# FrancisGregoryNg/Gaussian_Process_Optimization

Measured on AMD Instinct MI355X. Metric: GP fit+predict iters/sec at N=16384 D=8, higher is better.
Workload: dtype f64; 1 GPU; C3 (BASELINE.json configs[2]): N=16384, D=8 RBF iso, fit (K, Cholesky, alpha, LML) + predict mean/var at M=10000 candidates + EI arg-best; candidates_total=10000, candidates_this_rank=10000, entry_point=gp_fit_predict, kernel=RBF, fit=replicated on every rank (does not shard, SURVEY.md 8e), torch_imported=False, launcher=single process, emulate_fp64=0

## Files before the change

### gaussian_process_optimization_amd/_lib.py

```python
import ctypes
import os

import numpy as np

_HERE = os.path.dirname(os.path.abspath(__file__))
LIB_PATH = os.path.join(_HERE, "libgphip.so")

c_double_p = ctypes.POINTER(ctypes.c_double)
c_int64_p = ctypes.POINTER(ctypes.c_int64)
c_int_p = ctypes.POINTER(ctypes.c_int)

GP_KERNEL_RBF, GP_KERNEL_MATERN52 = 0, 1
GP_KERNEL_MATERN32, GP_KERNEL_EXPONENTIAL = 2, 3
GP_ACQ_EI, GP_ACQ_LCB, GP_ACQ_MPI = 0, 1, 2
GP_ERR_ARG, GP_ERR_HIP, GP_ERR_STATE, GP_ERR_RCCL, GP_ERR_NOT_PD_DIAG = -1, -2, -3, -4, -5

_vp = ctypes.c_void_p
SIGNATURES = [
    ("gp_last_error", ctypes.c_char_p, []),
    ("gp_version", ctypes.c_char_p, []),
    ("gp_device_count", ctypes.c_int, [c_int_p]),
    ("gp_device_info", ctypes.c_int, [ctypes.c_int, ctypes.c_char_p, ctypes.c_int, c_int_p, c_int64_p]),
    ("gp_create", ctypes.c_int, [ctypes.POINTER(_vp), ctypes.c_int]),
    ("gp_destroy", ctypes.c_int, [_vp]),
# ... 95 lines not shown
    ("gp_comm_info", ctypes.c_int, [_vp, c_int_p, c_int_p]),
    ("gp_comm_allgather_best", ctypes.c_int, [_vp, ctypes.c_double, ctypes.c_int64, c_double_p, c_int64_p]),
    ("gp_comm_bcast_fit", ctypes.c_int, [_vp, ctypes.c_int]),
    ("gp_comm_version", ctypes.c_int, [c_int_p]),
    ("gp_comm_selftest_fit_record", ctypes.c_int, [c_double_p, c_double_p, c_int_p]),
    ("gp_group_create", ctypes.c_int, [ctypes.POINTER(_vp), ctypes.c_int, c_int_p]),
    ("gp_group_destroy", ctypes.c_int, [_vp]),
    ("gp_group_info", ctypes.c_int, [_vp, c_int_p, c_int_p, ctypes.c_char_p, ctypes.c_int]),
    ("gp_group_member", ctypes.c_int, [_vp, ctypes.c_int, ctypes.POINTER(_vp)]),
    ("gp_group_set_data", ctypes.c_int, [_vp, c_double_p, c_double_p, ctypes.c_int64, ctypes.c_int, ctypes.c_int]),
    ("gp_group_set_params", ctypes.c_int, [_vp, ctypes.c_int, ctypes.c_int, ctypes.c_double, c_double_p, ctypes.c_double]),
    ("gp_group_set_gower", ctypes.c_int, [_vp, ctypes.c_int, c_int_p, c_double_p]),
    ("gp_group_set_option", ctypes.c_int, [_vp, ctypes.c_char_p, ctypes.c_int64]),
    ("gp_group_fit", ctypes.c_int, [_vp, ctypes.c_int, c_double_p, c_double_p, c_double_p]),
    ("gp_group_fmin", ctypes.c_int, [_vp, c_double_p]),
    ("gp_group_set_candidates", ctypes.c_int, [_vp, c_double_p, ctypes.c_int64]),
    ("gp_group_acq_argbest", ctypes.c_int, [_vp, ctypes.c_int, ctypes.c_double, ctypes.c_double, ctypes.c_double,
                                            ctypes.c_double, ctypes.c_int, c_int64_p, c_double_p]),
    ("gp_group_acq_lp_argbest", ctypes.c_int, [_vp, ctypes.c_int, ctypes.c_double, ctypes.c_double, ctypes.c_double,
                                               ctypes.c_double, ctypes.c_int, c_double_p, ctypes.c_int, c_double_p, c_double_p,
                                               ctypes.c_int, c_int64_p, ctypes.c_int, c_int64_p, c_double_p]),
    ("gp_group_acq_topk", ctypes.c_int, [_vp, ctypes.c_int, ctypes.c_double, ctypes.c_double, ctypes.c_double,
                                         ctypes.c_double, ctypes.c_int, ctypes.c_int, c_int64_p, c_double_p]),
    ("gp_merge_best", ctypes.c_int, [ctypes.c_int, c_double_p, c_int64_p, ctypes.c_int, c_int64_p, c_double_p]),
    ("gp_merge_topk", ctypes.c_int, [ctypes.c_int, c_double_p, c_int64_p, ctypes.c_int, ctypes.c_int, c_int64_p, c_double_p]),
    ("gp_last_phases", ctypes.c_int, [_vp, ctypes.c_int, ctypes.POINTER(ctypes.c_char_p), c_double_p, c_double_p,
                                      c_double_p]),
    ("gp_profile", ctypes.c_int, [_vp, ctypes.c_int]),
    ("gp_gemm_stats", ctypes.c_int, [_vp, c_int64_p, c_double_p, c_double_p]),
    ("gp_rns_stats", ctypes.c_int, [_vp, c_int64_p, c_double_p, c_double_p]),
    ("gp_gemm_busy", ctypes.c_int, [_vp, c_double_p]),
    ("gp_gemm_trace", ctypes.c_int, [_vp, ctypes.c_int, c_int64_p, c_int_p, c_double_p]),
    ("gp_synchronize", ctypes.c_int, [_vp]),
    ("gp_set_option", ctypes.c_int, [_vp, ctypes.c_char_p, ctypes.c_int64]),
]

_lib = None


def load_library():
    global _lib
    if _lib is not None:
        return _lib
    if not os.path.exists(LIB_PATH):
        raise RuntimeError(
            "libgphip.so is missing at %s: build it with `python -c 'import __graft_entry__ as g; g.build()'` "
            "(hipcc --offload-arch=gfx950). There is no CPU fallback." % LIB_PATH)
    lib = ctypes.CDLL(LIB_PATH)
    for name, restype, argtypes in SIGNATURES:
        fn = getattr(lib, name)
        fn.restype = restype
        fn.argtypes = argtypes
    _lib = lib
    return lib


def load():
    lib = load_library()
    n = ctypes.c_int(0)
    rc = lib.gp_device_count(ctypes.byref(n))
    if rc != 0 or n.value < 1:
        raise RuntimeError("gphip: no HIP device visible (%s). The GP path runs on MI355X only; "
                           "there is no CPU fallback." % lib.gp_last_error().decode())
    return lib


# ... 636 lines not shown

    def profile(self, on=True):
        check(self.lib, self.lib.gp_profile(self.h, int(on)), "gp_profile")

    def gemm_stats(self):
        n, ms, fl = ctypes.c_int64(), ctypes.c_double(), ctypes.c_double()
        check(self.lib, self.lib.gp_gemm_stats(self.h, ctypes.byref(n), ctypes.byref(ms), ctypes.byref(fl)),
              "gp_gemm_stats")
        return dict(launches=n.value, ms=ms.value, flops=fl.value)

    def rns_stats(self):
        n, ms, ops = ctypes.c_int64(), ctypes.c_double(), ctypes.c_double()
        check(self.lib, self.lib.gp_rns_stats(self.h, ctypes.byref(n), ctypes.byref(ms), ctypes.byref(ops)), "gp_rns_stats")
        return dict(launches=n.value, ms=ms.value, ops=ops.value)

    def gemm_busy(self):
        b = ctypes.c_double()
        check(self.lib, self.lib.gp_gemm_busy(self.h, ctypes.byref(b)), "gp_gemm_busy")
        return b.value

    def gemm_trace(self, cap=100000):
        tiles = np.empty(cap, dtype=np.int64)
        K = np.empty(cap, dtype=np.int32)
        ms = np.empty(cap)
        n = self.lib.gp_gemm_trace(self.h, cap, tiles.ctypes.data_as(c_int64_p), K.ctypes.data_as(c_int_p), dptr(ms))
        return tiles[:n], K[:n], ms[:n]

    def synchronize(self):
        check(self.lib, self.lib.gp_synchronize(self.h), "gp_synchronize")

    def set_option(self, name, value):
        check(self.lib, self.lib.gp_set_option(self.h, name.encode(), int(value)), "gp_set_option")

    def comm_unique_id(self):
        buf = ctypes.create_string_buffer(128)
        check(self.lib, self.lib.gp_comm_unique_id(buf), "gp_comm_unique_id")
        return buf.raw

    def comm_version(self):
        v = ctypes.c_int()
        check(self.lib, self.lib.gp_comm_version(ctypes.byref(v)), "gp_comm_version")
        return v.value

    def comm_init(self, uid, rank, nranks):
        check(self.lib, self.lib.gp_comm_init(self.h, uid, int(rank), int(nranks)), "gp_comm_init")

    def comm_info(self):
        r, n = ctypes.c_int(), ctypes.c_int()
        check(self.lib, self.lib.gp_comm_info(self.h, ctypes.byref(r), ctypes.byref(n)), "gp_comm_info")
        return r.value, n.value

    def comm_allgather_best(self, val, idx, nranks):
        vals = np.empty(nranks)
        idxs = np.empty(nranks, dtype=np.int64)
        check(self.lib, self.lib.gp_comm_allgather_best(self.h, float(val), int(idx), dptr(vals),
                                                        idxs.ctypes.data_as(c_int64_p)), "gp_comm_allgather_best")
        return vals, idxs

    def comm_allgather_topk(self, vals, idxs, nranks):
        vals = as_f64(vals, 1)
        idxs = np.ascontiguousarray(idxs, dtype=np.int64)
        k = vals.size
        av = np.empty(nranks * k)
        ai = np.empty(nranks * k, dtype=np.int64)
        check(self.lib, self.lib.gp_comm_allgather_topk(self.h, k, dptr(vals), idxs.ctypes.data_as(c_int64_p), dptr(av),
                                                        ai.ctypes.data_as(c_int64_p)), "gp_comm_allgather_topk")
# ... 106 lines not shown
```

### gaussian_process_optimization_amd/csrc/api_core.hip

```cpp
#include "api_internal.h"

thread_local std::string g_err;

static thread_local bool g_note_set = false;
static thread_local std::string g_note_msg;

int fail(int code, const char *fmt, ...) {
    char buf[512];
    va_list ap;
    va_start(ap, fmt);
    vsnprintf(buf, sizeof buf, fmt, ap);
    va_end(ap);
    g_err = buf;
    if (g_note_set) {
        g_err += " [after: " + g_note_msg + "]";
        g_note_set = false;
    }
    return code;
}

void gp_note_hip(hipError_t e, const char *what, const char *file, int line) {
    if (e == hipSuccess || g_note_set) return;
    char buf[512];
    snprintf(buf, sizeof buf, "%s -> %s (%s:%d)", what, hipGetErrorString(e), file, line);
    g_note_msg = buf;
    g_note_set = true;
}
int gp_pending_error() {
    if (!g_note_set) return 0;
    g_note_set = false;
    return fail(GP_ERR_HIP, "%s", g_note_msg.c_str());
}
void gp_clear_stale_note() { g_note_set = false; }
// ... 64 lines not shown
            int rp = reserve;
            if (const char *e = getenv("GPHIP_PRED_RESERVE")) rp = atoi(e);
            rc = make_bulk_stream(device, rp, &d.pred);
            if (rc) return rc;
        }
    }
    *out = d;
    return 0;
}

int phase_begin(gp_ctx *g, const char *name, double flops, double bytes) {
    if (g->nphases >= MAX_PHASES) return -1;
    Phase &p = g->phases[g->nphases];
    p.name = name;
    p.flops = flops;
    p.bytes = bytes;
    if (!p.used) {
        hipEventCreate(&p.e0);
        hipEventCreate(&p.e1);
        p.used = true;
    }
    GP_NOTE(hipEventRecord(p.e0, g->s));
    return g->nphases++;
}
void phase_end(gp_ctx *g, int id) {
    if (id >= 0) GP_NOTE(hipEventRecord(g->phases[id].e1, g->s));
}

void gemm(gp_ctx *g, hipStream_t s, int mode, double *C, long ldc, const double *A, long lda, const double *B, long ldb, int b_mul, int K, TileSet ts, const GemmOpt &o) {
    if (o.batch <= 0 || o.members <= 0) return;
    const long n = tileset_count(ts) * (o.batch / o.members), n_all = tileset_count(ts) * o.batch;
    if (n <= 0 || K <= 0) return;
    GemmOpt oo = o;
    if (n >= 1024 && !oo.stagger) oo.stagger = g->stagger;
    if (n >= 1024 && g->waves8) oo.waves8 = 1;
    if (oo.inplace && g->trsm_rows64 && !oo.waves8) oo.rows64 = g->trsm_rows64;
    const int small_thr = (s == g->s_panel) ? g->chain_small_below : g->small_below;
    if (small_thr > 0 && n < small_thr && !oo.inplace) oo.small = 1;
    if (g->pair_tri && (oo.small || (oo.waves8 && g->pair_tri >= 2)) && o.k_end_tri && !ts.tri && !o.tile_list && ts.c1 - ts.c0 >= 2)
        oo.pair = 1;
    hipEvent_t e0 = nullptr, e1 = nullptr;
    const bool small_sym = mode == 1 && oo.small && !oo.pair && !oo.rows64;
    const bool timed = g->profiling && (g->profile_class == 1 ? small_sym :
                       (n >= g->profile_min_tiles &&
                        (g->profile_min_tiles < 1024 || (mode == 1 && oo.waves8 && !oo.small))));
    if (timed) {
        if (g->gemm_ev_used + 2 > g->gemm_events.size()) {
            hipEvent_t a, b;
            hipEventCreate(&a);
            hipEventCreate(&b);
            g->gemm_events.push_back(a);
            g->gemm_events.push_back(b);
        }
        e0 = g->gemm_events[g->gemm_ev_used++];
        e1 = g->gemm_events[g->gemm_ev_used++];
        GP_NOTE(hipEventRecord(e0, s));
        g->gemm_tiles.push_back(n_all);
        g->gemm_K.push_back((o.k_tri || o.k_end_tri) ? -K : K);
    }
    if (g->supertile > 1 && !o.tile_list && !o.k_end_tri && o.batch == 1 && tileset_count(ts) >= 2048) {
        const std::array<int, 5> key{ts.r0, ts.r1, ts.c0, ts.c1, ts.tri};
        auto it = g->tile_lists.find(key);
        if (it == g->tile_lists.end()) {
            std::vector<short> l = build_tile_list(ts, g->supertile);
            DevBuf<short> d;
            if (d.alloc((long)l.size()) == hipSuccess) {
                hipMemcpy(d, l.data(), l.size() * sizeof(short), hipMemcpyHostToDevice);
                it = g->tile_lists.emplace(key, std::move(d)).first;
// ... 159 lines not shown
    delete g;
    return 0;
}

enum OptShape { OPT_RANGE, OPT_FLOOR, OPT_BOOL, OPT_RAW };
struct OptDesc {
    const char *name;
    int gp_ctx::*field;
    OptShape shape;
    int lo, hi;
};
static const OptDesc g_options[] = {
    {"panel_tiles", &gp_ctx::panel_tiles, OPT_RANGE, 1, 64},
    {"inner_tiles", &gp_ctx::inner_tiles, OPT_RANGE, 1, 2},
    {"inner_min_rows", &gp_ctx::inner_min_rows, OPT_FLOOR, 0},
    {"own_keep_per_row", &gp_ctx::own_keep_per_row, OPT_FLOOR, 0},
    {"own_keep_pipe_pct", &gp_ctx::own_keep_pipe_pct, OPT_RANGE, 0, 400},
    {"own_keep_base", &gp_ctx::own_keep_base, OPT_FLOOR, 0},
    {"lookahead", &gp_ctx::lookahead, OPT_BOOL},
    {"lookahead_min_tiles", &gp_ctx::lookahead_min_tiles, OPT_FLOOR, 0},
    {"pipe_start_pct", &gp_ctx::pipe_start_pct, OPT_RANGE, -1, 100},
    {"small_below", &gp_ctx::small_below, OPT_RAW},
    {"pipe_stages_grad", &gp_ctx::pipe_stages_grad, OPT_FLOOR, 0},
    {"pipe_start_pct_grad", &gp_ctx::pipe_start_pct_grad, OPT_RANGE, 0, 100},
    {"pipe_stages", &gp_ctx::pipe_stages, OPT_FLOOR, 0},
    {"lauum_panels", &gp_ctx::lauum_panels, OPT_RAW},
    {"side_alpha", &gp_ctx::side_alpha, OPT_RAW},
    {"pair_panels", &gp_ctx::pair_panels, OPT_BOOL},
    {"pair_tri", &gp_ctx::pair_tri, OPT_RAW},
    {"fmin_direct", &gp_ctx::fmin_direct, OPT_RAW},
    {"chain_small_below", &gp_ctx::chain_small_below, OPT_RAW},
    {"waves8", &gp_ctx::waves8, OPT_BOOL},
    {"stagger", &gp_ctx::stagger, OPT_RAW},
    {"trsm_rows64", &gp_ctx::trsm_rows64, OPT_RAW},
    {"rns_group_fit", &gp_ctx::rns_group_fit, OPT_RANGE, 1, 16},
    {"rns_group", &gp_ctx::rns_group, OPT_RANGE, 1, 16},
    {"emulate_fit", &gp_ctx::emulate_fit, OPT_BOOL},
    {"emulate_fp64", &gp_ctx::emulate_fp64, OPT_BOOL},
    {"rows_build", &gp_ctx::rows_build, OPT_RANGE, -1, 1},
    {"rows_nt", &gp_ctx::rows_nt, OPT_RANGE, -1, 1},
    {"rows_wide", &gp_ctx::rows_wide, OPT_BOOL},
};

static int store_option(gp_ctx *g, const OptDesc &o, int64_t value) {
    if (o.shape == OPT_RANGE && (value < o.lo || value > o.hi))
        return fail(GP_ERR_ARG, "%s out of range [%d, %d]", o.name, o.lo, o.hi);
    if (o.shape == OPT_FLOOR && value < o.lo) return fail(GP_ERR_ARG, "%s < %d", o.name, o.lo);
    if (o.shape == OPT_FLOOR) value = std::min<int64_t>(value, 1 << 20);
    if (o.shape == OPT_BOOL) value = value ? 1 : 0;
    g->*o.field = (int)value;
    return 0;
}

extern "C" int gp_set_option(gp_t *g, const char *name, int64_t value) {
    if (!g || !name) return fail(GP_ERR_ARG, "null argument");
    GP_DEAD_CHECK(g);
    for (const OptDesc &o : g_options) {
        if (strcmp(name, o.name)) continue;
        int rc = store_option(g, o, value);
        if (rc) return rc;
        if (o.field == &gp_ctx::lauum_panels) {
            g->wi_valid = false;
            g->li_valid = false;
            g->rows_calls_since_fit = 0;
            g->w_in_t2 = false;
        } else if (o.field == &gp_ctx::fmin_direct) {
// ... 4 lines not shown
        return 0;
    }
    if (!strcmp(name, "profile_min_tiles")) {
        if (value < 0) return fail(GP_ERR_ARG, "profile_min_tiles < 0");
        g->profile_min_tiles = value;
    } else if (!strcmp(name, "supertile")) {
        if (value < 0 || value > 64) return fail(GP_ERR_ARG, "supertile out of range");
        if (g->supertile != (int)value) {
            HIPCHK(hipSetDevice(g->device));
            HIPCHK(hipDeviceSynchronize());
            g->tile_lists.clear();
        }
        g->supertile = (int)value;
    } else if (!strcmp(name, "reserve_cus")) {
        if (value != g->bulk_reserved)
            return fail(GP_ERR_ARG, "reserve_cus is fixed when the device's streams are created (%d); set GPHIP_RESERVE_CUS "
                                    "before the first gp_create", g->bulk_reserved);
    } else if (!strcmp(name, "rns_interleave")) {
        rns_set_interleave((int)value);
    } else if (!strcmp(name, "debug_potrf_lds")) {
        if (value < 0 || value > (1 << 20)) return fail(GP_ERR_ARG, "debug_potrf_lds out of range");
        potrf_set_debug_lds((int)value);
    } else if (!strcmp(name, "debug_rows_skew")) {
        g->rows_counter_base += (unsigned int)value;
    } else if (!strcmp(name, "small_m")) {
        if (value < 0 || value > 8) return fail(GP_ERR_ARG, "small_m out of range (0..8)");
        g->small_m = value;
        g->predicted = false;
    } else if (!strcmp(name, "mc_max")) {
        if (value < GP_TILE) return fail(GP_ERR_ARG, "mc_max < 128");
        g->mc_max = round_up(value, GP_TILE);
    } else
        return fail(GP_ERR_ARG, "unknown option %s", name);
    return 0;
}

extern "C" int gp_synchronize(gp_t *g) {
    if (!g) return fail(GP_ERR_ARG, "null gp");
    GP_DEAD_CHECK(g);
    HIPCHK(hipSetDevice(g->device));
    GP_SYNC(g->s_panel);
    if (g->s_bulk) GP_SYNC(g->s_bulk);
    if (g->s_inv) GP_SYNC(g->s_inv);
    if (g->s_pred) GP_SYNC(g->s_pred);
    GP_SYNC(g->s);
    return 0;
}

extern "C" int gp_set_data(gp_t *g, const double *X, const double *Y, int64_t N, int D, int P) {
    if (!g || !X || !Y) return fail(GP_ERR_ARG, "null argument");
    GP_DEAD_CHECK(g);
    if (N < 1 || D < 1 || D > GP_MAX_D || P < 1 || P > GP_MAX_RHS)
        return fail(GP_ERR_ARG, "bad shape N=%ld D=%d P=%d (D <= %d, P <= %d)", (long)N, D, P, GP_MAX_D, GP_MAX_RHS);
    if (g->warp.n > 0 && P != 1)
        return fail(GP_ERR_STATE, "an output warp is on (gp_set_output_warp): it takes P = 1, switch it off before data with P = %d", P);
    HIPCHK(hipSetDevice(g->device));
    GP_SYNC(g->s);
    const long Npad = round_up(N, GP_TILE);
    if (Npad > g->capN || P > g->capP || !g->dA) {
        for (DevBuf<double> *b : {&g->dX, &g->dY, &g->dA, &g->dInvL, &g->dAlpha, &g->dW, &g->dMu}) b->release();
        const long capN = Npad;
        const int capP = std::max(P, g->capP);
        int rc;
        if ((rc = g->dX.reserve(capN * GP_MAX_D))) return rc;
        if ((rc = g->dY.reserve(capN * capP))) return rc;
        if ((rc = g->dA.reserve((capN + GP_MAX_RHS) * capN))) return rc;
// ... 164 lines not shown
```

### gaussian_process_optimization_amd/csrc/api_internal.h

```cpp
#pragma once
#include "gphip_internal.h"
#include "warp_math.h"
#include "../../include/gphip.h"

#include <hip/hip_ext.h>
#include <rccl/rccl.h>

#include <algorithm>
#include <array>
#include <cmath>
#include <cstdarg>
#include <cstdio>
#include <cstdlib>
#include <cstring>
#include <functional>
#include <map>
#include <mutex>
#include <set>
#include <string>
#include <type_traits>
#include <vector>

extern thread_local std::string g_err;
int fail(int code, const char *fmt, ...);
// ... 234 lines not shown
    int invp_W = 0;
    DevBuf<double> dDm, dDv, dDacq;
    int panel_tiles = 6;
    int lookahead = 1;
    int inner_min_rows = 0;
    int own_keep_per_row = 36, own_keep_base = 200;
    int own_keep_pipe_pct = 0;
    int inner_tiles = 1;
    int lookahead_min_tiles = 40;
    int reserve_cus = 32;
    long mc_max = 16384;
    long small_m = 8;
    Phase phases[MAX_PHASES];
    int nphases = 0;
    bool profiling = false;
    int profile_class = 0;
    std::vector<hipEvent_t> gemm_events;
    std::vector<hipEvent_t> rns_events;
    size_t rns_ev_used = 0;
    double rns_ops = 0.0;
    std::vector<long> gemm_tiles;
    std::map<std::array<int, 5>, DevBuf<short>> tile_lists;
    int supertile = 8;
    int small_below = 1400;
    int chain_small_below = 400;
    int lauum_panels = 1;
    int side_alpha = 1;
    int pair_panels = 1;
    int pair_tri = 2;
    int fmin_direct = 0;
    int trsm_rows64 = 32;
    int waves8 = 1;
    int stagger = 3;
    int pipe_stages_grad = 0, pipe_start_pct_grad = 40;
    int pipe_stages = 0;
    int pipe_done = 0;
    int pipe_start_pct = -1;
    std::vector<int> gemm_K;
    size_t gemm_ev_used = 0;
    long gemm_launches = 0;
    double gemm_flops = 0.0;
    double gemm_flops_all = 0.0;
    long profile_min_tiles = 1024;
    ncclComm_t comm = nullptr;
    int rank = 0, nranks = 1;
    DevBuf<double> dComm;
    int emulate_fp64 = 0;
    int rns_group = 8;
    int rns_group_fit = 8;
    DevBuf<signed char> dLr, dSr, dRr;
    DevBuf<signed char> dRm;
    DevBuf<signed char> dWr;
    std::vector<char> lr_done;
    int lr_W = 0, lr_e = 0;
    double jitter_try = 0.0;
    int emulate_fit = 1;
    bool emu_off_call = false;
    long emu_fallbacks = 0;
    DevBuf<double> dBatch;
    DevBuf<signed char> dBatchAux;
    WarpParams warp{0, 1.0, {}, {}, {}};
    DevBuf<double> dYraw;
    double warp_logjac = 0.0;
    DevBuf<double> dWarp;
    SparseState sp;
    EnsState ens;
// ... 159 lines not shown
```

### gaussian_process_optimization_amd/csrc/gemm.hip

```cpp
#include "gphip_internal.h"
#include <algorithm>

#define BK 16
#define LSTR 18

typedef unsigned v2u_t __attribute__((ext_vector_type(2)));
__device__ __forceinline__ double buf_load_f64(__amdgpu_buffer_rsrc_t r, unsigned voff, unsigned soff) {
    const v2u_t v = __builtin_amdgcn_raw_buffer_load_b64(r, voff, soff, 0);
    return __hiloint2double((int)v[1], (int)v[0]);
}
__device__ __forceinline__ void buf_store_f64(__amdgpu_buffer_rsrc_t r, unsigned voff, unsigned soff, double d) {
    v2u_t v;
    v[0] = (unsigned)__double2loint(d);
    v[1] = (unsigned)__double2hiint(d);
    __builtin_amdgcn_raw_buffer_store_b64(v, r, voff, soff, 0);
}

struct GemmArgs {
    double *C;
    long ldc;
    const double *A;
    long lda;
    const double *B;
    long ldb;
    int b_mul;
    int K;
    int r0, r1, c0, c1, tri;
    int k_tri;
    int k_sub;
    int k_end_tri;
    int b_sub;
    long sC, sA, sB;
    const short *tile_list;
    int stagger;
    int pair;
};

__device__ __forceinline__ void tile_from_linear(long t, const GemmArgs &a, int &i, int &c) {
    if (!a.tri) {
        int nr = a.r1 - a.r0;
        c = (int)(t / nr);
        c = a.k_end_tri ? a.c1 - 1 - c : a.c0 + c;
        i = a.r0 + (int)(t % nr);
        return;
    }
    const long H = a.r1 - a.c0;
    const double b = 2.0 * (double)H + 1.0;
    long j = (long)((b - sqrt(b * b - 8.0 * (double)t)) * 0.5);
    if (j < 0) j = 0;
    long S = j * H - j * (j - 1) / 2;
    while (S > t) {
        --j;
        S = j * H - j * (j - 1) / 2;
    }
    while (S + (H - j) <= t) {
        S += (H - j);
        ++j;
    }
    c = a.c0 + (int)j;
    i = c + (int)(t - S);
}

template <int MODE, int BT, int NWN, bool PAIR = false, int BM = BT>
__global__ __launch_bounds__(128 * NWN, (BT == 128 ? (BM < BT ? 2 : NWN) : 4)) void gemm_nt_kernel(GemmArgs a) {
    constexpr int NTH = 128 * NWN;
    constexpr int MT = BM / 32;
    constexpr int NT = BT / NWN / 16;
    constexpr int WT = BM / 2;
    constexpr int WTN = BT / NWN;
    constexpr int LQA = BM * 8 / NTH;
    constexpr int LQ = BT * 8 / NTH;
    constexpr int LR = NTH / 8;
    constexpr int SBUF = (BM + BT) * LSTR;
    __shared__ __attribute__((aligned(16))) double smem[2 * SBUF];

    const long nwg = gridDim.x, bid = blockIdx.x;
    const long q8 = nwg >> 3, r8 = nwg & 7, xcd = bid & 7;
    long wg = (xcd < r8 ? xcd * (q8 + 1) : r8 * (q8 + 1) + (xcd - r8) * q8) + (bid >> 3);
    int sub = 0;
    if (BT == 64) {
        sub = (int)(wg & 3);
        wg >>= 2;
    } else if (BM < BT) {
        sub = (int)(wg % (BT / BM));
        wg /= (BT / BM);
    }

    int ti, tc, tc2 = -1;
    if (PAIR) {
        const int nr = a.r1 - a.r0;
        const int cp = (int)(wg / nr);
        ti = a.r0 + (int)(wg % nr);
        tc = a.c1 - 1 - cp;
        tc2 = a.c0 + cp;
    } else if (a.tile_list) {
        ti = a.tile_list[2 * wg];
        tc = a.tile_list[2 * wg + 1];
// ... 65 lines not shown
#pragma unroll
    for (int q = 0; q < LQA; ++q) ra[q] = *(const double2_t *)(ap + q * a32);
#pragma unroll
    for (int q = 0; q < LQ; ++q) rb[q] = *(const double2_t *)(bp + q * b32);
    {
        double *As = smem, *Bs = smem + BM * LSTR;
#pragma unroll
        for (int q = 0; q < LQA; ++q) *(double2_t *)(As + soff + q * LR * LSTR) = ra[q];
#pragma unroll
        for (int q = 0; q < LQ; ++q) *(double2_t *)(Bs + soff + q * LR * LSTR) = rb[q];
    }
    __syncthreads();

    const int aoff = (wm * WT + li) * LSTR + lg * 4;
    const int boff = BM * LSTR + (wn * WTN + li) * LSTR + lg * 4;

    constexpr int PFA = PAIR ? 0 : ((BT == 128 && BM == 128 && NWN == 2) ? MT : 1);
    constexpr bool PF = PFA > 0;
    double2_t af[MT], bf[NT], pa_own[PF ? PFA : 1], pb_own[NT];
    double2_t *const pa = PF ? pa_own : af;
    double2_t *const pb = PF ? pb_own : bf;
    constexpr int PA = PF ? PFA : 1;
    {
        const double *as = smem + aoff, *bs = smem + boff;
#pragma unroll
        for (int m = 0; m < PA; ++m) pa[m] = *(const double2_t *)(as + m * 16 * LSTR);
#pragma unroll
        for (int n = 0; n < NT; ++n) pb[n] = *(const double2_t *)(bs + n * 16 * LSTR);
#pragma unroll
        for (int m = PA; m < MT; ++m) af[m] = *(const double2_t *)(as + m * 16 * LSTR);
    }
#define GP_MMA(A_, B_, m_, n_, e_) acc[m_][n_] = __builtin_amdgcn_mfma_f64_16x16x4f64((A_)[e_], (B_)[e_], acc[m_][n_], 0, 0, MODE == 1 ? 1 : 0)
#define GP_A1(m_) ((m_) < PA ? pa[m_] : af[m_])
    for (int kt = 0; kt < nk; ++kt) {
        const int buf = kt & 1;
        const bool more = (kt + 1 < nk);
        if (more) {
            ap += BK;
            bp += BK;
#pragma unroll
            for (int q = 0; q < LQA; ++q) ra[q] = *(const double2_t *)(ap + q * a32);
#pragma unroll
            for (int q = 0; q < LQ; ++q) rb[q] = *(const double2_t *)(bp + q * b32);
        }
        const double *as = smem + buf * SBUF + aoff;
        const double *bs = smem + buf * SBUF + boff;
#pragma unroll
        for (int m = 0; m < MT; ++m)
#pragma unroll
            for (int n = 0; n < NT; ++n) GP_MMA(GP_A1(m), pb[n], m, n, 0);
        if (PF) {
            __builtin_amdgcn_sched_barrier(0);
#pragma unroll
            for (int m = 0; m < PFA; ++m) af[m] = *(const double2_t *)(as + m * 16 * LSTR + 2);
#pragma unroll
            for (int n = 0; n < NT; ++n) bf[n] = *(const double2_t *)(bs + n * 16 * LSTR + 2);
            __builtin_amdgcn_sched_barrier(0);
        }
#pragma unroll
        for (int m = 0; m < MT; ++m)
#pragma unroll
            for (int n = 0; n < NT; ++n) GP_MMA(GP_A1(m), pb[n], m, n, 1);
        if (PF) __builtin_amdgcn_sched_barrier(0);
        if (!PF) {
            af[0] = *(const double2_t *)(as + 2);
#pragma unroll
// ... 20 lines not shown
#pragma unroll
                for (int m = 0; m < PFA; ++m) pa[m] = *(const double2_t *)(as2 + m * 16 * LSTR);
#pragma unroll
                for (int n = 0; n < NT; ++n) pb[n] = *(const double2_t *)(bs2 + n * 16 * LSTR);
            }
            __builtin_amdgcn_sched_barrier(0);
        }
#pragma unroll
        for (int m = 0; m < MT; ++m)
#pragma unroll
            for (int n = 0; n < NT; ++n) GP_MMA(af[m], bf[n], m, n, 1);
        if (PF) __builtin_amdgcn_sched_barrier(0);
        if (more) {
            if (!PF) {
                pa[0] = *(const double2_t *)(as2);
#pragma unroll
                for (int n = 0; n < NT; ++n) pb[n] = *(const double2_t *)(bs2 + n * 16 * LSTR);
            }
#pragma unroll
            for (int m = PA; m < MT; ++m) af[m] = *(const double2_t *)(as2 + m * 16 * LSTR);
        }
    }
#undef GP_A1
#undef GP_MMA

#pragma unroll
    for (int m = 0; m < MT; ++m)
#pragma unroll
        for (int n = 0; n < NT; ++n)
#pragma unroll
            for (int r = 0; r < 4; ++r)
                buf_store_f64(crs, cbyte + n * 128, (unsigned)(m * 16 + 4 * r) * crow, acc[m][n][r]);
    }
}

void launch_gemm_nt(hipStream_t s, int mode, double *C, long ldc, const double *A, long lda,
                    const double *B, long ldb, int b_mul, int K, TileSet ts, const GemmOpt &o) {
    long n = tileset_count(ts);
    if (n <= 0 || K <= 0 || o.batch <= 0) return;
    GemmArgs a;
    a.C = C; a.ldc = ldc; a.A = A; a.lda = lda; a.B = B; a.ldb = ldb;
    a.b_mul = b_mul; a.K = K;
    a.r0 = ts.r0; a.r1 = ts.r1; a.c0 = ts.c0; a.c1 = ts.c1; a.tri = ts.tri;
    a.k_tri = o.k_tri; a.k_sub = o.k_sub; a.k_end_tri = o.k_end_tri; a.b_sub = o.b_sub;
    a.sC = o.sC; a.sA = o.sA; a.sB = o.sB;
    a.tile_list = o.tile_list;
    a.stagger = o.stagger;
    a.pair = o.pair;
    if (o.small && o.pair) {
        const long np = (long)(ts.r1 - ts.r0) * ((ts.c1 - ts.c0 + 1) / 2);
        dim3 grid((unsigned)(4 * np), (unsigned)o.batch);
        if (mode == 0)
            GP_LAUNCH((gemm_nt_kernel<0, 64, 2, true>), grid, dim3(256), 0, s, a);
        else
            GP_LAUNCH((gemm_nt_kernel<1, 64, 2, true>), grid, dim3(256), 0, s, a);
    } else if (o.rows64 == 32) {
        dim3 grid((unsigned)(4 * n), (unsigned)o.batch);
        if (mode == 0)
            GP_LAUNCH((gemm_nt_kernel<0, 128, 2, false, 32>), grid, dim3(256), 0, s, a);
        else
            GP_LAUNCH((gemm_nt_kernel<1, 128, 2, false, 32>), grid, dim3(256), 0, s, a);
    } else if (o.rows64) {
        dim3 grid((unsigned)(2 * n), (unsigned)o.batch);
        if (mode == 0)
            GP_LAUNCH((gemm_nt_kernel<0, 128, 2, false, 64>), grid, dim3(256), 0, s, a);
        else
            GP_LAUNCH((gemm_nt_kernel<1, 128, 2, false, 64>), grid, dim3(256), 0, s, a);
    } else if (o.waves8 && o.pair) {
        const long np = (long)(ts.r1 - ts.r0) * ((ts.c1 - ts.c0 + 1) / 2);
        dim3 grid((unsigned)np, (unsigned)o.batch);
        if (mode == 0)
            GP_LAUNCH((gemm_nt_kernel<0, 128, 4, true>), grid, dim3(512), 0, s, a);
        else
            GP_LAUNCH((gemm_nt_kernel<1, 128, 4, true>), grid, dim3(512), 0, s, a);
    } else if (o.small) {
        dim3 grid((unsigned)(4 * n), (unsigned)o.batch);
        if (mode == 0)
            GP_LAUNCH((gemm_nt_kernel<0, 64, 2>), grid, dim3(256), 0, s, a);
        else
            GP_LAUNCH((gemm_nt_kernel<1, 64, 2>), grid, dim3(256), 0, s, a);
    } else if (o.waves8) {
        dim3 grid((unsigned)n, (unsigned)o.batch);
        if (mode == 0)
            GP_LAUNCH((gemm_nt_kernel<0, 128, 4>), grid, dim3(512), 0, s, a);
        else
            GP_LAUNCH((gemm_nt_kernel<1, 128, 4>), grid, dim3(512), 0, s, a);
    } else {
        dim3 grid((unsigned)n, (unsigned)o.batch);
        if (mode == 0)
            GP_LAUNCH((gemm_nt_kernel<0, 128, 2>), grid, dim3(256), 0, s, a);
        else
            GP_LAUNCH((gemm_nt_kernel<1, 128, 2>), grid, dim3(256), 0, s, a);
    }
}

std::vector<short> build_tile_list(const TileSet &ts, int S) {
    std::vector<short> out;
    const int c_lo = ts.c0, c_hi = ts.c1;
    const int r_lo = ts.tri ? ts.c0 : ts.r0, r_hi = ts.r1;
    for (int sc = c_lo; sc < c_hi; sc += S)
        for (int sr = (ts.tri ? sc : r_lo); sr < r_hi; sr += S)
            for (int c = sc; c < std::min(sc + S, c_hi); ++c)
                for (int i = sr; i < std::min(sr + S, r_hi); ++i) {
                    if (ts.tri && i < c) continue;
                    out.push_back((short)i);
                    out.push_back((short)c);
                }
    return out;
}
```

### gaussian_process_optimization_amd/csrc/gphip_internal.h

```cpp
#pragma once
#include <hip/hip_runtime.h>
#include <stdint.h>
#include <algorithm>
#include <string>
#include <vector>

#define GP_TILE 128
#define GP_MAX_RHS 128

typedef double double4_t __attribute__((ext_vector_type(4)));
typedef double double2_t __attribute__((ext_vector_type(2)));

void gp_note_hip(hipError_t e, const char *what, const char *file, int line);
#define GP_NOTE(call) gp_note_hip((call), #call, __FILE__, __LINE__)
#define GP_LAUNCH(kernel, grid, block, lds, stream, ...)                                   \
    do {                                                                                   \
        (void)hipGetLastError();  \
        hipLaunchKernelGGL(kernel, grid, block, lds, stream, __VA_ARGS__);                 \
        gp_note_hip(hipGetLastError(), #kernel, __FILE__, __LINE__);                       \
    } while (0)

#define GP_MAX_D 64
struct KernParams {
    int kernel;
// ... 70 lines not shown
        const bool zero = (r2 == 0.0);
        g = zero ? 0.0 : -k / (zero ? 1.0 : r);
    }
}
__device__ __forceinline__ void gp_k_and_g(int kernel, double variance, double r2, double &k, double &g) {
    if (GP_FAMILY_PAIR(kernel)) gp_k_and_g_pair<1>(kernel, variance, r2, k, g);
    else gp_k_and_g_pair<0>(kernel, variance, r2, k, g);
}

__host__ __device__ static inline double kp_div(const KernParams &kp, int d) { return kp.gower ? kp.gdiv[d] : kp.ls[d]; }

struct TileSet {
    int r0, r1, c0, c1, tri;
};
static inline long tileset_count(const TileSet &t) {
    if (!t.tri) return (long)(t.r1 - t.r0) * (t.c1 - t.c0);
    long n = 0;
    for (int c = t.c0; c < t.c1; ++c) n += (t.r1 - c) > 0 ? (t.r1 - c) : 0;
    return n;
}

struct GemmOpt {
    int k_tri = 0;
    int k_sub = 0;
    int k_end_tri = 0;
    int b_sub = 0;
    int batch = 1;
    int members = 1;
    long sC = 0, sA = 0, sB = 0;
    const short *tile_list = nullptr;
    int stagger = 0;
    int small = 0;
    int waves8 = 0;
    int inplace = 0;
    int rows64 = 0;
    int pair = 0;
};
std::vector<short> build_tile_list(const TileSet &ts, int S);
void launch_gemm_nt(hipStream_t s, int mode, double *C, long ldc, const double *A, long lda,
                    const double *B, long ldb, int b_mul, int K, TileSet ts, const GemmOpt &o = GemmOpt());

void launch_potrf_tile(hipStream_t s, double *A, long lda, int t, double *invL, int *info, int nb = 1, long sA = 0, long sI = 0,
                       int sInfo = 0);
void launch_potrf_pair(hipStream_t s, double *A, long lda, int t, double *invL, int *info);
void launch_trsm2(hipStream_t s, double *A, long lda, int t, const double *invL, int r0, int r1);
void potrf_set_debug_lds(int bytes);


void launch_kbuild(hipStream_t s, double *A, long lda, const double *X, long N, long Npad, const KernParams &kp, double diag_add,
                   int full, int nb = 1, long sA = 0, const KernParams *kpt = nullptr, const double *diag_tab = nullptr);
void launch_set_rhs(hipStream_t s, double *A, long lda, const double *Y, long N, long Npad, int P, int nb = 1, long sA = 0);
void launch_cross_k(hipStream_t s, double *T, long ldt, const double *Xs, long M, long Mpad,
                    const double *X, long N, long Npad, const KernParams &kp);

void launch_cross_k_rows(hipStream_t s, double *T, long ldt, const double *Xs, int M, const double *X, long N, long Npad,
                         const KernParams &kp);

void launch_logdet(hipStream_t s, const double *A, long lda, long N, double *out, int nb = 1, long sA = 0, long so = 0);
void launch_rhs_sumsq(hipStream_t s, const double *A, long lda, long N, long Npad, int P, double *out);

void launch_trsv_backward(hipStream_t s, const double *L, long lda, const double *invP, int W, long Npad, const double *Z, long ldz,
                          int P, double *Aout, double *w, int nb = 1, long sL = 0, long sP = 0, long sV = 0);

void launch_predict_reduce(hipStream_t s, const double *T, long ldt, long M, long N, const double *Z,
                           long ldz, int P, double kss, double noise_add, double *mean, double *var);

// ... 140 lines not shown
```

### include/gphip.h

```cpp
#ifndef GPHIP_H
#define GPHIP_H

#include <stdint.h>

#ifdef __cplusplus
extern "C" {
#endif

typedef struct gp_ctx gp_t;

#define GP_KERNEL_RBF 0
#define GP_KERNEL_MATERN52 1
#define GP_KERNEL_MATERN32 2
#define GP_KERNEL_EXPONENTIAL 3

#define GP_ACQ_EI 0
#define GP_ACQ_LCB 1
#define GP_ACQ_MPI 2

#define GP_ERR_ARG (-1)
#define GP_ERR_HIP (-2)
#define GP_ERR_STATE (-3)
#define GP_ERR_RCCL (-4)
#define GP_ERR_NOT_PD_DIAG (-5)
// ... 153 lines not shown
int gp_sparse_set_candidates(gp_t *gp, const double *Xs, int64_t M);
int gp_sparse_acq(gp_t *gp, int type, double par, double fmin, double y_mean, double y_std, int lp, int transform,
                  const double *Xb, int nb, const double *r_x0, const double *s_x0, double *out, double *dout);
int gp_sparse_acq_argbest(gp_t *gp, int type, double par, double fmin, double y_mean, double y_std, int lp, int transform,
                          const double *Xb, int nb, const double *r_x0, const double *s_x0, int sense, const int64_t *exclude,
                          int nex, int64_t *idx, double *val);
int gp_sparse_acq_topk(gp_t *gp, int type, double par, double fmin, double y_mean, double y_std, int sense, int k, int64_t *idx,
                       double *val);

int gp_sparse_predict_rows(gp_t *gp, const double *Xs, int64_t M, int include_noise, double *mean, double *var, double *dmdx,
                           double *dvdx);
int gp_sparse_acq_rows(gp_t *gp, const double *Xs, int64_t M, int type, double par, double fmin, double y_mean, double y_std,
                       int lp, int transform, const double *Xb, int nb, const double *r_x0, const double *s_x0, double *out,
                       double *dout);
int gp_sparse_rows_stats(gp_t *gp, int64_t *fused, int64_t *fallback);


int gp_ens_fit(gp_t *gp, int S, const double *variance, const double *lengthscale, const double *noise, int maxtries, double *lml,
               double *logdet, double *jitter_used, double *fmin);
int gp_ens_info(gp_t *gp, int *S);
int gp_ens_predict_rows(gp_t *gp, const double *Xs, int64_t M, int include_noise, double *mean, double *var, double *dmdx,
                        double *dvdx);
int gp_ens_acq_rows(gp_t *gp, const double *Xs, int64_t M, int type, double par, double *out, double *dout);
int gp_ens_acq(gp_t *gp, int type, double par, double *out);
int gp_ens_acq_argbest(gp_t *gp, int type, double par, int sense, int64_t *idx, double *val);

int gp_last_phases(gp_t *gp, int cap, const char **names, double *ms, double *flops, double *bytes);
int gp_profile(gp_t *gp, int on);
int gp_gemm_stats(gp_t *gp, int64_t *launches, double *ms, double *flops);
int gp_rns_stats(gp_t *gp, int64_t *launches, double *ms, double *ops);
int gp_gemm_busy(gp_t *gp, double *busy_ms);
int gp_gemm_trace(gp_t *gp, int cap, int64_t *tiles, int *K, double *ms);
int gp_synchronize(gp_t *gp);
int gp_set_option(gp_t *gp, const char *name, int64_t value);

#ifdef __cplusplus
}
#endif
#endif
```

Baseline: 14.85 fit+predict iters/s.

## Add hand-scheduled 8-wave FP64 MFMA GEMM main loop with sched barriers

Adds a specialized GEMM kernel variant for the 8-wave 128x128 tile case. Its K loop explicitly interleaves MFMA instructions with LDS loads and stores and global prefetches, using scheduling barriers to fix the order. The aim is to hide memory latency behind matrix math in the Cholesky trailing updates and kernel-matrix GEMMs. It is enabled by default on the main stream. A debug GEMM entry point and options for the tile threshold are also added. The risk is that the hand-written schedule raises register pressure, or is worse than the compiler's own ordering.

After: 15.05 fit+predict iters/s, median of 6. +1.3%, better.

```diff
diff --git a/gaussian_process_optimization_amd/_lib.py b/gaussian_process_optimization_amd/_lib.py
--- a/gaussian_process_optimization_amd/_lib.py
+++ b/gaussian_process_optimization_amd/_lib.py
@@ -151,6 +151,8 @@
     ("gp_gemm_busy", ctypes.c_int, [_vp, c_double_p]),
     ("gp_gemm_trace", ctypes.c_int, [_vp, ctypes.c_int, c_int64_p, c_int_p, c_double_p]),
     ("gp_synchronize", ctypes.c_int, [_vp]),
+    ("gp_debug_gemm", ctypes.c_int, [_vp, ctypes.c_int, c_double_p, c_double_p, c_double_p, ctypes.c_int64, ctypes.c_int,
+                                     ctypes.c_int, ctypes.c_int, ctypes.c_int, ctypes.c_int, ctypes.c_int]),
     ("gp_set_option", ctypes.c_int, [_vp, ctypes.c_char_p, ctypes.c_int64]),
 ]
 
@@ -853,6 +855,16 @@
     def set_option(self, name, value):
         check(self.lib, self.lib.gp_set_option(self.h, name.encode(), int(value)), "gp_set_option")
 
+    def debug_gemm(self, mode, C, A, B, K, r0, r1, c0, c1, tri=False):
+        A, B = as_f64(A, 2), as_f64(B, 2)
+        out = np.array(C, dtype=np.float64, order="C")
+        ld = out.shape[1]
+        if A.shape != (r1 * 128, ld) or B.shape != (c1 * 128, ld) or out.shape[0] != r1 * 128:
+            raise ValueError("C, A [r1 * 128, ld] and B [c1 * 128, ld] share one pitch")
+        check(self.lib, self.lib.gp_debug_gemm(self.h, int(mode), dptr(out), dptr(A), dptr(B), ld, int(K), int(r0), int(r1),
+                                               int(c0), int(c1), int(bool(tri))), "gp_debug_gemm")
+        return out
+
     def comm_unique_id(self):
         buf = ctypes.create_string_buffer(128)
         check(self.lib, self.lib.gp_comm_unique_id(buf), "gp_comm_unique_id")
diff --git a/gaussian_process_optimization_amd/csrc/api_core.hip b/gaussian_process_optimization_amd/csrc/api_core.hip
--- a/gaussian_process_optimization_amd/csrc/api_core.hip
+++ b/gaussian_process_optimization_amd/csrc/api_core.hip
@@ -1,4 +1,6 @@
 #include "api_internal.h"
+
+#define BK_MIN 16
 
 thread_local std::string g_err;
 
@@ -129,8 +131,9 @@
     const long n = tileset_count(ts) * (o.batch / o.members), n_all = tileset_count(ts) * o.batch;
     if (n <= 0 || K <= 0) return;
     GemmOpt oo = o;
-    if (n >= 1024 && !oo.stagger) oo.stagger = g->stagger;
-    if (n >= 1024 && g->waves8) oo.waves8 = 1;
+    if (n >= g->long_min_tiles && !oo.stagger) oo.stagger = g->stagger;
+    if (n >= g->long_min_tiles && g->waves8) oo.waves8 = 1;
+    oo.sched = g->gemm_sched && (s == g->s || g->gemm_sched_side);
     if (oo.inplace && g->trsm_rows64 && !oo.waves8) oo.rows64 = g->trsm_rows64;
     const int small_thr = (s == g->s_panel) ? g->chain_small_below : g->small_below;
     if (small_thr > 0 && n < small_thr && !oo.inplace) oo.small = 1;
@@ -356,6 +359,9 @@
     {"chain_small_below", &gp_ctx::chain_small_below, OPT_RAW},
     {"waves8", &gp_ctx::waves8, OPT_BOOL},
     {"stagger", &gp_ctx::stagger, OPT_RAW},
+    {"gemm_sched", &gp_ctx::gemm_sched, OPT_BOOL},
+    {"gemm_sched_side", &gp_ctx::gemm_sched_side, OPT_BOOL},
+    {"long_min_tiles", &gp_ctx::long_min_tiles, OPT_FLOOR, 1},
     {"trsm_rows64", &gp_ctx::trsm_rows64, OPT_RAW},
     {"rns_group_fit", &gp_ctx::rns_group_fit, OPT_RANGE, 1, 16},
     {"rns_group", &gp_ctx::rns_group, OPT_RANGE, 1, 16},
@@ -426,6 +432,27 @@
         g->mc_max = round_up(value, GP_TILE);
     } else
         return fail(GP_ERR_ARG, "unknown option %s", name);
+    return 0;
+}
+
+extern "C" int gp_debug_gemm(gp_t *g, int mode, double *C, const double *A, const double *B, int64_t ld, int K, int r0, int r1,
+                             int c0, int c1, int tri) {
+    if (!g || !C || !A || !B) return fail(GP_ERR_ARG, "null argument");
+    GP_DEAD_CHECK(g);
+    if (mode < 0 || mode > 1 || K < BK_MIN || K % BK_MIN || r0 < 0 || r1 <= r0 || c0 < 0 || c1 <= c0 || r1 > 256 || c1 > 256 ||
+        (tri && r1 <= c1 - 1) || ld % 2 || ld < K || ld < (int64_t)c1 * GP_TILE)
+        return fail(GP_ERR_ARG, "gp_debug_gemm: bad shape (mode %d K %d rows %d..%d columns %d..%d ld %ld)", mode, K, r0, r1, c0, c1, (long)ld);
+    HIPCHK(hipSetDevice(g->device));
+    const long ra = (long)r1 * GP_TILE, rb = (long)c1 * GP_TILE;
+    DevBuf<double> dC, dA, dB;
+    int rc;
+    if ((rc = dC.reserve(ra * ld)) || (rc = dA.reserve(ra * ld)) || (rc = dB.reserve(rb * ld))) return rc;
+    HIPCHK(hipMemcpyAsync(dC, C, (size_t)(ra * ld) * sizeof(double), hipMemcpyHostToDevice, g->s));
+    HIPCHK(hipMemcpyAsync(dA, A, (size_t)(ra * ld) * sizeof(double), hipMemcpyHostToDevice, g->s));
+    HIPCHK(hipMemcpyAsync(dB, B, (size_t)(rb * ld) * sizeof(double), hipMemcpyHostToDevice, g->s));
+    gemm(g, g->s, mode, dC, ld, dA, ld, dB, ld, 1, K, TileSet{r0, r1, c0, c1, tri ? 1 : 0});
+    HIPCHK(hipMemcpyAsync(C, dC, (size_t)(ra * ld) * sizeof(double), hipMemcpyDeviceToHost, g->s));
+    GP_SYNC(g->s);
     return 0;
 }
 
diff --git a/gaussian_process_optimization_amd/csrc/api_internal.h b/gaussian_process_optimization_amd/csrc/api_internal.h
--- a/gaussian_process_optimization_amd/csrc/api_internal.h
+++ b/gaussian_process_optimization_amd/csrc/api_internal.h
@@ -290,6 +290,9 @@
     int trsm_rows64 = 32;
     int waves8 = 1;
     int stagger = 3;
+    int gemm_sched = 1;
+    int gemm_sched_side = 0;
+    int long_min_tiles = 1024;
     int pipe_stages_grad = 0, pipe_start_pct_grad = 40;
     int pipe_stages = 0;
     int pipe_done = 0;
diff --git a/gaussian_process_optimization_amd/csrc/gemm.hip b/gaussian_process_optimization_amd/csrc/gemm.hip
--- a/gaussian_process_optimization_amd/csrc/gemm.hip
+++ b/gaussian_process_optimization_amd/csrc/gemm.hip
@@ -1,5 +1,6 @@
 #include "gphip_internal.h"
 #include <algorithm>
+#include <type_traits>
 
 #define BK 16
 #define LSTR 18
@@ -61,8 +62,8 @@
     i = c + (int)(t - S);
 }
 
-template <int MODE, int BT, int NWN, bool PAIR = false, int BM = BT>
-__global__ __launch_bounds__(128 * NWN, (BT == 128 ? (BM < BT ? 2 : NWN) : 4)) void gemm_nt_kernel(GemmArgs a) {
+template <int MODE, int BT, int NWN, bool PAIR, int BM, bool SCHED>
+__device__ __forceinline__ void gemm_nt_body(const GemmArgs &a) {
     constexpr int NTH = 128 * NWN;
     constexpr int MT = BM / 32;
     constexpr int NT = BT / NWN / 16;
@@ -194,6 +195,74 @@
     }
 #define GP_MMA(A_, B_, m_, n_, e_) acc[m_][n_] = __builtin_amdgcn_mfma_f64_16x16x4f64((A_)[e_], (B_)[e_], acc[m_][n_], 0, 0, MODE == 1 ? 1 : 0)
 #define GP_A1(m_) ((m_) < PA ? pa[m_] : af[m_])
+    if constexpr (SCHED) {
+        static_assert(MT == 4 && NT == 2 && LQA == 2 && LQ == 2 && PA == 1 && PF && !PAIR, "schedule written for the 8-wave 128x128 instance");
+#define GP_F __builtin_amdgcn_sched_barrier(0)
+#define GP_S1(m_, n_, e_) GP_MMA(GP_A1(m_), pb[n_], m_, n_, e_)
+#define GP_S2(m_, n_, e_) GP_MMA(af[m_], bf[n_], m_, n_, e_)
+#define GP_LD(p_) (*(const double2_t *)(p_))
+        const double *as = smem + aoff, *bs = smem + boff;
+        double *Aw = smem + SBUF + soff;
+        int flip = SBUF;
+        auto stage = [&](auto w_, auto l_) __attribute__((always_inline)) {
+            constexpr bool W = decltype(w_)::value;
+            constexpr bool L = decltype(l_)::value;
+            double *const Bw = Aw + BM * LSTR;
+            GP_S1(0, 0, 0); GP_F; af[0] = GP_LD(as + 2); GP_F;
+            GP_S1(0, 1, 0); GP_F; bf[0] = GP_LD(bs + 2); GP_F;
+            GP_S1(1, 0, 0); GP_F; bf[1] = GP_LD(bs + 16 * LSTR + 2); GP_F;
+            GP_S1(1, 1, 0); GP_S1(2, 0, 0); GP_S1(2, 1, 0); GP_S1(3, 0, 0); GP_S1(3, 1, 0); GP_F;
+            GP_S1(1, 0, 1); GP_F; if (W) *(double2_t *)(Aw) = ra[0]; GP_F;
+            GP_S1(1, 1, 1); GP_F; af[1] = GP_LD(as + 16 * LSTR + 2); GP_F;
+            GP_S1(2, 0, 1); GP_F; if (W) *(double2_t *)(Aw + LR * LSTR) = ra[1]; GP_F;
+            GP_S1(2, 1, 1); GP_F; af[2] = GP_LD(as + 32 * LSTR + 2); GP_F;
+            GP_S1(3, 0, 1); GP_F; if (W) *(double2_t *)(Bw) = rb[0]; GP_F;
+            GP_S1(3, 1, 1); GP_F; af[3] = GP_LD(as + 48 * LSTR + 2); GP_F;
+            GP_S1(0, 0, 1); GP_F; if (W) *(double2_t *)(Bw + LR * LSTR) = rb[1]; GP_F;
+            GP_S1(0, 1, 1); GP_F;
+            GP_S2(0, 0, 0); GP_F;
+            if (W) {
+                __syncthreads();
+                as += flip;
+                bs += flip;
+                Aw -= flip;
+                flip = -flip;
+            }
+            const double *const as2 = as, *const bs2 = bs;
+            if (L) { ap += BK; bp += BK; }
+            GP_F; if (L) ra[0] = GP_LD(ap); GP_F;
+            GP_S2(0, 1, 0); GP_F; if (L) ra[1] = GP_LD(ap + a32); GP_F;
+            GP_S2(1, 0, 0); GP_F; if (L) rb[0] = GP_LD(bp); GP_F;
+            GP_S2(1, 1, 0); GP_F; if (L) rb[1] = GP_LD(bp + b32); GP_F;
+            GP_S2(2, 0, 0); GP_F; if (W) pa[0] = GP_LD(as2); GP_F;
+            GP_S2(2, 1, 0); GP_F; if (W) pb[0] = GP_LD(bs2); GP_F;
+            GP_S2(3, 0, 0); GP_F; if (W) pb[1] = GP_LD(bs2 + 16 * LSTR); GP_F;
+            GP_S2(3, 1, 0); GP_F;
+            GP_S2(1, 0, 1); GP_S2(1, 1, 1); GP_F; if (W) af[1] = GP_LD(as2 + 16 * LSTR); GP_F;
+            GP_S2(2, 0, 1); GP_S2(2, 1, 1); GP_F; if (W) af[2] = GP_LD(as2 + 32 * LSTR); GP_F;
+            GP_S2(3, 0, 1); GP_S2(3, 1, 1); GP_F; if (W) af[3] = GP_LD(as2 + 48 * LSTR); GP_F;
+            GP_S2(0, 0, 1); GP_S2(0, 1, 1); GP_F;
+        };
+        if (nk > 1) {
+            ap += BK;
+            bp += BK;
+            ra[0] = GP_LD(ap); ra[1] = GP_LD(ap + a32);
+            rb[0] = GP_LD(bp); rb[1] = GP_LD(bp + b32);
+        }
+        using Y = std::true_type;
+        using N = std::false_type;
+        int kt = 0;
+        for (; kt + 2 < nk; ++kt) stage(Y{}, Y{});
+        if (kt + 1 < nk) {
+            stage(Y{}, N{});
+            ++kt;
+        }
+        if (kt < nk) stage(N{}, N{});
+#undef GP_LD
+#undef GP_S2
+#undef GP_S1
+#undef GP_F
+    } else
     for (int kt = 0; kt < nk; ++kt) {
         const int buf = kt & 1;
         const bool more = (kt + 1 < nk);
@@ -280,6 +349,15 @@
             for (int r = 0; r < 4; ++r)
                 buf_store_f64(crs, cbyte + n * 128, (unsigned)(m * 16 + 4 * r) * crow, acc[m][n][r]);
     }
+}
+
+template <int MODE, int BT, int NWN, bool PAIR = false, int BM = BT>
+__global__ __launch_bounds__(128 * NWN, (BT == 128 ? (BM < BT ? 2 : NWN) : 4)) void gemm_nt_kernel(GemmArgs a) {
+    gemm_nt_body<MODE, BT, NWN, PAIR, BM, false>(a);
+}
+template <int MODE>
+__global__ __launch_bounds__(512, 4) void gemm_nt_sched_kernel(GemmArgs a) {
+    gemm_nt_body<MODE, 128, 4, false, 128, true>(a);
 }
 
 void launch_gemm_nt(hipStream_t s, int mode, double *C, long ldc, const double *A, long lda,
@@ -327,6 +405,12 @@
             GP_LAUNCH((gemm_nt_kernel<0, 64, 2>), grid, dim3(256), 0, s, a);
         else
             GP_LAUNCH((gemm_nt_kernel<1, 64, 2>), grid, dim3(256), 0, s, a);
+    } else if (o.waves8 && o.sched) {
+        dim3 grid((unsigned)n, (unsigned)o.batch);
+        if (mode == 0)
+            GP_LAUNCH((gemm_nt_sched_kernel<0>), grid, dim3(512), 0, s, a);
+        else
+            GP_LAUNCH((gemm_nt_sched_kernel<1>), grid, dim3(512), 0, s, a);
     } else if (o.waves8) {
         dim3 grid((unsigned)n, (unsigned)o.batch);
         if (mode == 0)
diff --git a/gaussian_process_optimization_amd/csrc/gphip_internal.h b/gaussian_process_optimization_amd/csrc/gphip_internal.h
--- a/gaussian_process_optimization_amd/csrc/gphip_internal.h
+++ b/gaussian_process_optimization_amd/csrc/gphip_internal.h
@@ -126,6 +126,7 @@
     int stagger = 0;
     int small = 0;
     int waves8 = 0;
+    int sched = 0;
     int inplace = 0;
     int rows64 = 0;
     int pair = 0;
diff --git a/include/gphip.h b/include/gphip.h
--- a/include/gphip.h
+++ b/include/gphip.h
@@ -209,6 +209,8 @@
 int gp_gemm_busy(gp_t *gp, double *busy_ms);
 int gp_gemm_trace(gp_t *gp, int cap, int64_t *tiles, int *K, double *ms);
 int gp_synchronize(gp_t *gp);
+int gp_debug_gemm(gp_t *gp, int mode, double *C, const double *A, const double *B, int64_t ld, int K, int r0, int r1, int c0,
+                  int c1, int tri);
 int gp_set_option(gp_t *gp, const char *name, int64_t value);
 
 #ifdef __cplusplus
```
